# SLIDE-3D/SLIDE

Hardware: AMD Instinct MI355X
Metric: latent shapes/sec (pos+feat DDPM, 1000 steps, 16 pts) (higher is better)
Workload: dtype f16 (MFMA operands + activation storage; f32 accumulate, norm statistics, softmax); position DDPM: two-term f16 operand splits (fp32-grade); 1 GPU; BASELINE configs[1]+[2]: airplane position DDPM (16x3) + chair feature DDPM (16x51), batch 256 per GPU; 1 step = one reverse step of each; shape = 1000+1000 steps; batch_per_gpu=256, prec=fp16, pos_prec=split, replay=eager, pos_batch_multiple=2, pos_stream_cus=176, prime_steps=0, finite=True

## Files before the change

### slide_amd/csrc/ddpm_update.h

```cpp
#pragma once
#include "gemm_common.h"

namespace {

__device__ __forceinline__ void philox_round(uint32_t &c0, uint32_t &c1, uint32_t &c2, uint32_t &c3, uint32_t k0,
                                             uint32_t k1) {
  const uint64_t p0 = (uint64_t)0xD2511F53u * c0, p1 = (uint64_t)0xCD9E8D57u * c2;
  const uint32_t n0 = (uint32_t)(p1 >> 32) ^ c1 ^ k0, n1 = (uint32_t)p1, n2 = (uint32_t)(p0 >> 32) ^ c3 ^ k1,
                 n3 = (uint32_t)p0;
  c0 = n0; c1 = n1; c2 = n2; c3 = n3;
}
__device__ __forceinline__ float philox_normal(uint32_t seed_lo, uint32_t seed_hi, uint32_t step, uint32_t elem,
                                               uint32_t nonce) {
  uint32_t c0 = elem, c1 = step, c2 = 0x243F6A88u ^ nonce, c3 = 0x85A308D3u, k0 = seed_lo, k1 = seed_hi;
#pragma unroll
  for (int i = 0; i < 10; ++i) {
    philox_round(c0, c1, c2, c3, k0, k1);
    k0 += 0x9E3779B9u; k1 += 0xBB67AE85u;
  }
  const float u1 = ((float)(c0 >> 8) + 0.5f) * (1.0f / 16777216.0f);
  const float u2 = ((float)(c1 >> 8) + 0.5f) * (1.0f / 16777216.0f);
  return sqrtf(-2.0f * logf(u1)) * cosf(6.28318530717958647692f * u2);
}

__device__ __forceinline__ void advance_t_last_block(int *t_dev, int t, int step) {
  __syncthreads();
  if (threadIdx.x == 0) {
    __threadfence();
    if (atomicAdd(&t_dev[2], 1) == (int)gridDim.x - 1) {
      t_dev[2] = 0;
      t_dev[0] = t - 1;
      t_dev[1] = step + 1;
    }
  }
}

__device__ __forceinline__ void update_feat_element(int e, int npts, int C, int kdim, int eps_ld, float clamp,
                                                    uint32_t seed_lo, uint32_t seed_hi, float *__restrict__ x,
                                                    const float *__restrict__ eps, const float *__restrict__ noise, int t,
                                                    int step, uint32_t nonce, uint32_t eoff, const float *__restrict__ complete_x0,
                                                    const float *__restrict__ kmask, const float *__restrict__ keypoint,
                                                    const float *__restrict__ rc, const float *__restrict__ rm1,
                                                    const float *__restrict__ c1, const float *__restrict__ c2,
                                                    const float *__restrict__ stdv, void *__restrict__ feat0 = nullptr,
                                                    int ldf = 0, int half_out = 0,
                                                    const SlidePrepCopy *__restrict__ copies = nullptr, int n_copies = 0,
                                                    float eps_val = 0.f,
                                                    const float *z_pre = nullptr) {
#pragma clang fp contract(off)
  if (e >= npts * C) return;
  const int p = e / C, c = e - p * C;
  if (c < kdim) {
    x[e] = keypoint[(size_t)p * kdim + c];
    return;
  }
  const float xv = x[e];
  float x0 = rc[t] * xv - rm1[t] * (eps ? eps[eps_ld ? (size_t)p * eps_ld + c : (size_t)e] : eps_val);
  if (clamp > 0.f) x0 = fminf(fmaxf(x0, -clamp), clamp);
  if (complete_x0) {
    const float m = kmask[p];
    x0 = x0 * m + complete_x0[e] * (1.f - m);
  }
// ... 25 lines not shown
```

### slide_amd/csrc/engine.hip

```cpp
#include "gemm_common.h"
#include "gemm_small.h"
#include "ddpm_update.h"

#include <cstdlib>

int slide_launch_rows_op(const SlideOp &o, hipStream_t s);
#ifdef SLIDE_EXPERIMENTS
int slide_launch_gemm_xs(const GemmArgs &a, int npxl, int cbw, bool aff, bool gat, int want_occ, hipStream_t s);
#endif
int slide_launch_gemm_gx(const SlideOp &o, hipStream_t s);
int slide_launch_gemm_gxs(const SlideOp &o, hipStream_t s);
int slide_launch_attn_tail_split(const SlideOp &o, hipStream_t s);
int slide_launch_point_chain(const SlideOp &o, hipStream_t s);
int slide_launch_pp_stage(const SlideOp &o, hipStream_t s);
int slide_launch_pair_norm(const SlideOp &o, hipStream_t s);
int slide_launch_sa_chain(const SlideOp &o, hipStream_t s);
int slide_launch_block_body(const SlideOp &o, hipStream_t s);
#ifdef SLIDE_EXPERIMENTS
int slide_launch_gemm_chain(const SlideOp &o, hipStream_t s);
#endif
#define SLIDE_ST_EXPERIMENT (-20)
int slide_launch_gemm_gx_dual(const SlideOp &o, hipStream_t s);
int slide_launch_sa_chain_p(const SlideOp &o, hipStream_t s);

namespace {

template <int PREC, int NPXL, int CBW, bool PAIRRES = false>
__global__ __launch_bounds__(256, (PREC == SLIDE_PREC_SPLIT && NPXL == 4) ? 1 : 2) void gemm_kernel(GemmArgs a) {
  using T = typename TileT<PREC>::T;
  constexpr int LDK = TileT<PREC>::LDK;
  constexpr int EPL = TileT<PREC>::EPL;
  constexpr int TPR = BK / EPL;
  constexpr int RPP = 256 / TPR;
  constexpr int TN = 32 * CBW;
  constexpr int XP = TM / RPP, WP = TN / RPP;
  extern __shared__ __attribute__((aligned(16))) unsigned char smem_raw[];
  constexpr bool SPLIT = PREC == SLIDE_PREC_SPLIT;
// ... 1636 lines not shown
                  w3 = w[(size_t)(k + 3) * n_o + j], w4 = w[(size_t)(k + 4) * n_o + j], w5 = w[(size_t)(k + 5) * n_o + j],
                  w6 = w[(size_t)(k + 6) * n_o + j], w7 = w[(size_t)(k + 7) * n_o + j];
      a0 += in[k] * w0; a1 += in[k + 1] * w1_; a2 += in[k + 2] * w2_; a3 += in[k + 3] * w3;
      a0 += in[k + 4] * w4; a1 += in[k + 5] * w5; a2 += in[k + 6] * w6; a3 += in[k + 7] * w7;
    }
    return (a0 + a1) + (a2 + a3);
  };
  for (int j = tid; j < H; j += 256) h1[j] = swishf(b1[j] + gemv(emb, t_dim, w1, H, j));
  __syncthreads();
  for (int j = tid; j < H; j += 256) h2[j] = swishf(b2[j] + gemv(h1, H, w2, H, j));
  __syncthreads();
  for (int j = tid; j < n_out; j += 256) out[(size_t)b * n_out + j] = bfc[j] + gemv(h2, H, wfc, n_out, j);
}

__global__ __launch_bounds__(256) void cond_kernel(int dim, int n_out, const int64_t *__restrict__ label,
                                                   const float *__restrict__ class_emb, const float *__restrict__ wfc,
                                                   const float *__restrict__ bfc, float *__restrict__ out) {
  extern __shared__ float sm[];
  const int b = blockIdx.x, tid = threadIdx.x;
  const float *ce = class_emb + (size_t)label[b] * dim;
  for (int k = tid; k < dim; k += 256) sm[k] = ce[k];
  __syncthreads();
  for (int j = tid; j < n_out; j += 256) {
    float acc = bfc[j];
    for (int k = 0; k < dim; ++k) acc += sm[k] * wfc[(size_t)k * n_out + j];
    out[(size_t)b * n_out + j] = acc;
  }
}

__global__ __launch_bounds__(256) void update_pos_kernel(int n, int eps_ld, uint32_t seed_lo, uint32_t seed_hi, float *__restrict__ x,
                                                         const float *__restrict__ eps, const float *__restrict__ noise,
                                                         int *__restrict__ t_dev, const float *__restrict__ c_eps,
                                                         const float *__restrict__ sqrt_alpha,
                                                         const float *__restrict__ sigma) {
#pragma clang fp contract(off)
  const int e = blockIdx.x * 256 + threadIdx.x;
  const int t = t_dev[0], step = t_dev[1];
  if (e < n) {
    const int ep = eps_ld ? (e / 3) * eps_ld + e % 3 : e;
    float v = (x[e] - c_eps[t] * eps[ep]) / sqrt_alpha[t];
    if (t > 0) {
      const float z = noise ? noise[(size_t)step * n + e]
                            : philox_normal(seed_lo, seed_hi, (uint32_t)step, (uint32_t)e + (uint32_t)t_dev[4] * 48u, (uint32_t)t_dev[3]);
      v = v + sigma[t] * z;
    }
    x[e] = v;
  }
  advance_t_last_block(t_dev, t, step);
}

__global__ __launch_bounds__(256) void update_feat_kernel(int npts, int C, int kdim, int eps_ld, float clamp, uint32_t seed_lo,
                                                          uint32_t seed_hi, float *__restrict__ x,
                                                          const float *__restrict__ eps, const float *__restrict__ noise,
                                                          int *__restrict__ t_dev, const float *__restrict__ keypoint,
                                                          const float *__restrict__ rc, const float *__restrict__ rm1,
                                                          const float *__restrict__ c1, const float *__restrict__ c2,
                                                          const float *__restrict__ stdv,
                                                          const float *__restrict__ complete_x0,
                                                          const float *__restrict__ kmask, void *__restrict__ feat0, int ldf,
                                                          int half_out, const SlidePrepCopy *__restrict__ copies, int n_copies) {
#pragma clang fp contract(off)
  const int t = t_dev[0], step = t_dev[1];
  const uint32_t nonce = (uint32_t)t_dev[3];
  const uint32_t eoff = (uint32_t)t_dev[4] * (uint32_t)(16 * C);
#pragma unroll
  for (int j = 0; j < 4; ++j)
    update_feat_element(blockIdx.x * 1024 + j * 256 + threadIdx.x, npts, C, kdim, eps_ld, clamp, seed_lo, seed_hi, x, eps, noise,
                        t, step, nonce, eoff, complete_x0, kmask, keypoint, rc, rm1, c1, c2, stdv, feat0, ldf, half_out, copies,
                        n_copies);
  advance_t_last_block(t_dev, t, step);
}

typedef SlideHeadArgs HeadArgs;

template <int K0MAX>
__global__ __launch_bounds__(256, 2) void head_update_kernel(HeadArgs a) {
#pragma clang fp contract(off)
  using T = _Float16;
  constexpr int LDX = K0MAX + 8, LDH = 128 + 8;
  __shared__ __attribute__((aligned(16))) T xs[64 * LDX];
  __shared__ __attribute__((aligned(16))) T hs[64 * LDH];
  const int tid = threadIdx.x, lane = tid & 63, wave = tid >> 6, half = lane >> 5, col = lane & 31;
  const int row0 = blockIdx.x * 64;
  const int t = a.t_dev[0], step = a.t_dev[1];
  const uint32_t nonce = (uint32_t)a.t_dev[3];
  const uint32_t eoff = (uint32_t)a.t_dev[4] * (uint32_t)(16 * a.C);
  const int nk0 = a.k0 >> 4;
  f16x8 w0[K0MAX / 16];
  {
    const GLOBAL_AS T *wp = gptr<const T>((uint64_t)a.W0) + (size_t)(wave * 32 + col) * a.k0 + half * 8;
#pragma unroll
    for (int s2 = 0; s2 < K0MAX / 16; ++s2)
      if (s2 < nk0) w0[s2] = *(const GLOBAL_AS f16x8 *)(wp + s2 * 16);
  }
  const int cb2 = a.n1c == 2 ? (wave & 1) : 0, rb2 = a.n1c == 2 ? (wave >> 1) : wave;
  const bool l2 = rb2 < 2;
  f16x8 w1[8];
  if (l2) {
    const GLOBAL_AS T *wp = gptr<const T>((uint64_t)a.W1) + (size_t)(cb2 * 32 + col) * 128 + half * 8;
#pragma unroll
    for (int s2 = 0; s2 < 8; ++s2) w1[s2] = *(const GLOBAL_AS f16x8 *)(wp + s2 * 16);
  }
  {
// ... 302 lines not shown
    a.add_bs = (int)o.f[2];
    a.add_n = (int)o.f[3] >> 1;
    a.aff_relu = (int)o.f[3] & 1;
  }
  a.at_V = o.p[5]; a.at_out = o.p[6]; a.at_counts = (const int *)o.p[7]; a.at_vss = (const float *)o.p[8];
  a.rows = o.i[0]; a.x_ld = o.i[1]; a.k_pad = o.i[2]; a.n_cob = o.i[3]; a.in_bs = o.i[5];
  resolve_epi(a);
  const int K = o.i[4];
  a.at_ldv = o.i[6]; a.at_ldo = o.i[7]; a.at_pps = o.i[8] > 0 ? o.i[8] : 1; a.at_vrelu = o.i[9]; a.at_C = o.i[10];
  a.at_klog2 = K == 4 ? 2 : K == 8 ? 3 : K == 16 ? 4 : K == 32 ? 5 : -1;
  if (a.at_klog2 < 0 || a.rows <= 0 || a.rows % K || a.k_pad % BK || a.x_ld % 8 || a.n_cob <= 0 || !a.X || !a.W || !a.epi || !a.at_V ||
      !a.at_out || a.at_ldv % 4 || a.at_ldo % 4 || a.at_ldv < a.n_cob * 32 || a.at_ldo < a.n_cob * 32 || (a.in_scale && !a.in_shift))
    return -3;
  return a.in_scale ? launch_gemm_attend<true>(a, s) : launch_gemm_attend<false>(a, s);
}

int run_gemm(const SlideOp &o, hipStream_t s) {
  GemmArgs a;
  a.X = o.p[0]; a.W = o.p[1]; a.epi = (const SlideEpi *)o.p[2];
  a.in_scale = (const float *)o.p[3]; a.in_shift = (const float *)o.p[4];
  a.in_add = nullptr; a.aff_relu = 0; a.add_bs = 0; a.add_n = 0; a.aff_tps = 1;
  if (a.in_scale && !o.p[8]) {
    a.in_add = (const float *)o.p[11];
    a.aff_tps = (int)o.f[1] > 1 ? (int)o.f[1] : 1;
    a.add_bs = (int)o.f[2];
    a.add_n = (int)o.f[3] >> 1;
    a.aff_relu = (int)o.f[3] & 1;
  }
  a.dbg = (unsigned long long *)o.p[5];
  a.stagger = (int)(o.f[0] * 100.f);
  a.sched = (int *)o.p[7];
  a.gfeat = o.p[8]; a.gidx = (const int *)o.p[9];
  a.gn_fin = (const SlideGnFin *)o.p[6];
  a.gx_d2 = (const float *)o.p[12]; a.gx_w = (const float *)o.p[13];
  a.gx_ta = a.gx_tb = nullptr; a.gx_vv = nullptr; a.gx_add_idx = nullptr;
  a.g_nsplit = (int)o.f[1]; a.g_ldf = (int)o.f[2]; a.g_klog2 = (int)o.f[3];
  a.rows = o.i[0]; a.x_ld = o.i[1]; a.k_pad = o.i[2]; a.n_cob = o.i[3]; a.in_bs = o.i[5];
  a.ch_epi = nullptr; a.ch_n_cob = 0;
  resolve_epi(a);
  const int npxl = o.i[4], prec = o.i[6], cbw = o.i[7], glds = o.i[8] & 1;
  a.w_cm = (o.i[8] >> 1) & 1;
  if ((o.i[8] >> 2) & 1) {
    if (prec == SLIDE_PREC_SPLIT && !glds && !a.in_scale && !o.p[8] && !o.p[10] && cbw == 2) {
      if (a.k_pad % BK || a.x_ld % 4 || a.rows <= 0 || a.n_cob <= 0) return -3;
      if (npxl == 8) return launch_gemm<SLIDE_PREC_SPLIT, 8, 2, true>(a, s);
      if (npxl == 7) return launch_gemm<SLIDE_PREC_SPLIT, 7, 2, true>(a, s);
      return -12;
    }
    if (!glds || prec != SLIDE_PREC_F16 || a.in_scale || o.p[8] || o.p[10]) return -12;
    if (npxl == 8) return launch_gemm_glds<8, 2, 3, 32, false, false, true>(a, s);
    if (npxl == 7) return launch_gemm_glds<7, 2, 3, 32, false, false, true>(a, s);
    return -12;
  }
  if (a.w_cm && (!glds || (npxl != 7 && npxl != 8) || o.p[10] || o.i[9] == 1)) return -11;
  if (a.k_pad % BK || a.x_ld % 8 || a.rows <= 0 || a.n_cob <= 0) return -3;
  if (prec == SLIDE_PREC_F16 && npxl == 4 && o.i[9] != 3 &&
      (!a.gn_fin || ((a.rows + 63) / 64) * ((a.n_cob + 1) / 2) <= 1024))
    return launch_gemm_small(a, s);
  if (a.gn_fin) return -10;
#ifndef SLIDE_EXPERIMENTS
  if (o.p[10]) return SLIDE_ST_EXPERIMENT;
#else
  if (o.p[10] && glds && prec == SLIDE_PREC_F16 && o.i[9] != 5 && (npxl == 8 || npxl == 7) && !(a.gfeat && a.in_scale)) {
    int st = -8;
    const bool aff = a.in_scale != nullptr, gat = a.gfeat != nullptr;
    st = slide_launch_gemm_xs(a, npxl, cbw, aff, gat, o.i[9] >= 11 && o.i[9] <= 13 ? o.i[9] - 10 : 0, s);
// ... 234 lines not shown
                     (const TT *)o.p[0], (const TT *)o.p[1], (TT *)o.p[2])
      if (o.i[5] == 16 && o.i[6] == SLIDE_PREC_F16) ATTN(16, _Float16);
      else if (o.i[5] == 16) ATTN(16, float);
      else if (o.i[5] == 8 && o.i[6] == SLIDE_PREC_F16) ATTN(8, _Float16);
      else if (o.i[5] == 8) ATTN(8, float);
      else return -5;
#undef ATTN
      break;
    }
    case SLIDE_OP_COPY_COLS: {
      if (o.i[0] <= 0 || o.i[1] <= 0) break;
      const dim3 g((o.i[0] * o.i[1] + 255) / 256), blk(256);
#define CPY(TS, TD)                                                                                               \
  hipLaunchKernelGGL((copy_cols_kernel<TS, TD>), g, blk, 0, s, o.i[0], o.i[1], o.i[2], o.i[3], (const TS *)o.p[0], \
                     (TD *)o.p[1])
      if (o.i[4] && o.i[5]) CPY(_Float16, _Float16);
      else if (o.i[4]) CPY(_Float16, float);
      else if (o.i[5]) CPY(float, _Float16);
      else CPY(float, float);
#undef CPY
      break;
    }
    case SLIDE_OP_TEMB:
      hipLaunchKernelGGL(temb_kernel, dim3(o.i[0]), dim3(256), (size_t)o.i[1] * 9 * sizeof(float), s, o.i[1], o.i[2],
                         (const float *)o.p[0], (const int *)o.p[1], (const float *)o.p[9], (const float *)o.p[2],
                         (const float *)o.p[3], (const float *)o.p[4], (const float *)o.p[5], (const float *)o.p[6],
                         (const float *)o.p[7], (float *)o.p[8]);
      break;
    case SLIDE_OP_COND:
      hipLaunchKernelGGL(cond_kernel, dim3(o.i[0]), dim3(256), (size_t)o.i[1] * sizeof(float), s, o.i[1], o.i[2],
                         (const int64_t *)o.p[0], (const float *)o.p[1], (const float *)o.p[2], (const float *)o.p[3],
                         (float *)o.p[4]);
      break;
    case SLIDE_OP_UPDATE_POS:
      hipLaunchKernelGGL(update_pos_kernel, dim3((o.i[0] + 255) / 256), dim3(256), 0, s, o.i[0], o.i[1], (uint32_t)o.i[2],
                         (uint32_t)o.i[3], (float *)o.p[0], (const float *)o.p[1], (const float *)o.p[2],
                         (int *)o.p[3], (const float *)o.p[4], (const float *)o.p[5], (const float *)o.p[6]);
      break;
    case SLIDE_OP_UPDATE_FEAT:
      hipLaunchKernelGGL(update_feat_kernel, dim3((o.i[0] * o.i[1] + 1023) / 1024), dim3(256), 0, s, o.i[0], o.i[1],
                         o.i[2], o.i[5], o.f[0], (uint32_t)o.i[3], (uint32_t)o.i[4], (float *)o.p[0], (const float *)o.p[1],
                         (const float *)o.p[2], (int *)o.p[3], (const float *)o.p[4], (const float *)o.p[5],
                         (const float *)o.p[6], (const float *)o.p[7], (const float *)o.p[8], (const float *)o.p[9],
                         (const float *)o.p[10], (const float *)o.p[11], o.p[12], o.i[6], o.i[7],
                         (const SlidePrepCopy *)o.p[13], o.i[8]);
      break;
#ifndef SLIDE_EXPERIMENTS
    case SLIDE_OP_HEAD_UPDATE:
    case SLIDE_OP_GEMM_CHAIN:
      return SLIDE_ST_EXPERIMENT;
#else
    case SLIDE_OP_GEMM_CHAIN:
      return slide_launch_gemm_chain(o, s);
    case SLIDE_OP_HEAD_UPDATE: {
      const SlideHeadArgs *h = (const SlideHeadArgs *)o.p[0];
      if (!h || h->rows <= 0 || h->rows % 16 || h->k0 % 32 || h->k0 <= 0 || h->k0 > 160 || h->x_ld < h->k0 || h->x_ld % 8 ||
          (h->n1c != 1 && h->n1c != 2) || !h->X || !h->W0 || !h->W1 || !h->v0 || !h->b1 || !h->x || !h->t_dev ||
          (h->kind != 0 && h->kind != 1) || h->C > 32 * h->n1c)
        return -3;
      const int grid = (h->rows + 63) / 64;
      if (h->k0 <= 96) hipLaunchKernelGGL(head_update_kernel<96>, dim3(grid), dim3(256), 0, s, *h);
      else hipLaunchKernelGGL(head_update_kernel<160>, dim3(grid), dim3(256), 0, s, *h);
      break;
    }
#endif
    case SLIDE_OP_POINT_CHAIN:
      return slide_launch_point_chain(o, s);
    case SLIDE_OP_GEMM_ATTEND:
      return run_gemm_attend(o, s);
    case SLIDE_OP_ATTN_TAIL:
      return ((int)o.f[1] & 8) ? slide_launch_attn_tail_split(o, s) : run_attn_tail(o, s);
    case SLIDE_OP_GEMM_GX:
      return (int)o.f[0] == 3 ? slide_launch_gemm_gxs(o, s) : slide_launch_gemm_gx(o, s);
    case SLIDE_OP_GEMM_GX_DUAL:
      return slide_launch_gemm_gx_dual(o, s);
    case SLIDE_OP_PAIR_NORM:
      return slide_launch_pair_norm(o, s);
    case SLIDE_OP_PP_STAGE:
      return slide_launch_pp_stage(o, s);
// ... 163 lines not shown
```

### slide_amd/csrc/gemm_common.h

```cpp
#pragma once
#include <hip/hip_runtime.h>
#include <stdint.h>

#include <type_traits>

#include "../../include/slide_engine.h"

typedef float f32x16 __attribute__((ext_vector_type(16)));
typedef _Float16 f16x8 __attribute__((ext_vector_type(8)));
typedef _Float16 f16x4 __attribute__((ext_vector_type(4)));
typedef _Float16 f16x2 __attribute__((ext_vector_type(2)));
typedef uint32_t u32x4 __attribute__((ext_vector_type(4)));
typedef float f32x2 __attribute__((ext_vector_type(2)));

struct GemmArgs {
  const void *X;
  const void *W;
  const SlideEpi *epi;
  const float *in_scale, *in_shift;
  const float *in_add;
  int aff_relu, add_bs, add_n, aff_tps;
  int rows, x_ld, k_pad, n_cob, in_bs;
  int w_cm;
  int shm_bytes;
  const SlideGnFin *gn_fin;
  const void *gfeat;
  const int *gidx;
  int g_ldf, g_nsplit, g_klog2;
  int *sched;
  int stagger;
  unsigned long long *dbg;
  const void *gx_ta, *gx_tb;
  const float *gx_d2, *gx_w, *gx_vv;
  const int *gx_add_idx;
  int gx_ld, gx_mode, gx_add_idx_stride, gx_vbs;
  const void *ch_W;
  const SlideEpi *ch_epi;
  int ch_n_cob, ch_k_pad;
  const float *vecs, *ch_vecs;
  const void *at_V;
  void *at_out;
  const float *at_vss;
  const int *at_counts;
  int at_ldv, at_ldo, at_klog2, at_pps, at_vrelu, at_C;
};

static inline void resolve_epi(GemmArgs &a) {
  a.vecs = a.ch_vecs = nullptr;
  if ((uintptr_t)a.epi & SLIDE_EPI_PACKED_VECS) {
    a.epi = reinterpret_cast<const SlideEpi *>((uintptr_t)a.epi & ~SLIDE_EPI_PACKED_VECS);
    a.vecs = reinterpret_cast<const float *>(a.epi + a.n_cob);
  }
  if ((uintptr_t)a.ch_epi & SLIDE_EPI_PACKED_VECS) {
    a.ch_epi = reinterpret_cast<const SlideEpi *>((uintptr_t)a.ch_epi & ~SLIDE_EPI_PACKED_VECS);
    a.ch_vecs = reinterpret_cast<const float *>(a.ch_epi + a.ch_n_cob);
  }
}

// ... 789 lines not shown
```

### slide_amd/csrc/gemm_small.h

```cpp
#pragma once
#include "gemm_common.h"

namespace {

template <int NST, bool AFF, int PAIR>
__device__ __forceinline__ void small_body(const GemmArgs &a, const PairArgs &pa, const int bid) {
  using T = _Float16;
  constexpr int NPXL = 4;
  constexpr int STAGE_B = 96 * 64;
  constexpr int NJ = 6;
  extern __shared__ __attribute__((aligned(16))) unsigned char smem_raw[];
  SLIDE_STAMP(a, 0);
  const int ntc = (a.n_cob + 1) / 2;
  const int tc = bid % ntc, tr = bid / ntc;
  const int row0 = tr * 64, cob0 = tc * 2;
  const int tid = threadIdx.x, lane = tid & 63, wave = tid >> 6;
  const int half = lane >> 5, col = lane & 31;
  const int kh = wave >> 1, cbw = wave & 1;
  unsigned char *const ring = smem_raw + (size_t)wave * NST * STAGE_B;
  uint32_t *const epi_lds = reinterpret_cast<uint32_t *>(smem_raw + (size_t)4 * NST * STAGE_B);
  float *const vec_lds = reinterpret_cast<float *>(epi_lds + 2 * EPI_DW + (2 * EPI_DW) % 4);
  const T *gp[NJ];
#pragma unroll
  for (int j = 0; j < NJ; ++j) {
// ... 30 lines not shown
  }
  const int nk = a.k_pad / 32;
  const int mine = nk > kh ? (nk - kh + 1) / 2 : 0;
#pragma unroll
  for (int s0 = 0; s0 < NST - 1; ++s0)
    if (s0 < mine) issue(kh + 2 * s0, s0);
  stage_epilogue_tables<2>(a, cob0, tid, epi_lds, vec_lds);
  float *const pair_lds = vec_lds + 2 * 96;
  float *const pair_ext = reinterpret_cast<float *>(smem_raw + 20480);
  int ext_n[2] = {0, 0};
  float ext_d[2] = {0.f, 0.f}, ext_w[2] = {0.f, 0.f};
  if constexpr (PAIR != 0) {
    const int nb = a.rows >> NPXL, b0 = row0 >> NPXL;
    if (tid < 192) {
      const int bb = b0 + tid / 48 < nb ? b0 + tid / 48 : nb - 1;
      pair_lds[tid] = pa.xyz[(size_t)bb * 48 + tid % 48];
    }
    if (PAIR == 2) {
#pragma unroll
      for (int u = 0; u < 2; ++u) {
        const int i = tid + 256 * u;
        const int bb = b0 + (i >> 7) < nb ? b0 + (i >> 7) : nb - 1, t = i & 127;
        const int slot = (bb * 16 + (t >> 3)) * 16 + (t & 7);
        ext_n[u] = pa.nbr[slot]; ext_d[u] = pa.d2t[slot]; ext_w[u] = pa.wt[slot];
      }
    }
  }
  _Float16 *const aff_lds = reinterpret_cast<_Float16 *>(vec_lds + 2 * 96);
  if (AFF) {
    const int nb = a.rows >> NPXL;
    if (a.gn_fin) {
      const SlideGnFin f = *a.gn_fin;
      const int off = (int)(a.in_scale - f.scale);
      float *const grp = reinterpret_cast<float *>(aff_lds + (size_t)4 * 2 * a.k_pad);
      if (tid < 128) {
        const int sm = tid >> 5, g = tid & 31;
        int b = (row0 >> NPXL) + sm;
        b = b < nb ? b : nb - 1;
        float mean = 0.f, rstd = 0.f;
        if (g < f.G) {
#pragma clang fp contract(off)
          float S = 0.f, SS = 0.f;
          typedef float f4u __attribute__((ext_vector_type(4), aligned(4)));
          const int c_end = f.gend[g];
          const float *ps = f.sum + (size_t)b * f.bs, *pq = f.sq + (size_t)b * f.bs;
          for (int cc = f.gstart[g]; cc < c_end; cc += 16) {
            f4u s4[4], q4[4];
            int base[4];
#pragma unroll
            for (int u = 0; u < 4; ++u) {
              base[u] = cc + 4 * u + 4 <= f.bs ? cc + 4 * u : f.bs - 4;
              s4[u] = *reinterpret_cast<const f4u *>(ps + base[u]);
              q4[u] = *reinterpret_cast<const f4u *>(pq + base[u]);
            }
#pragma unroll
            for (int u = 0; u < 4; ++u)
#pragma unroll
              for (int e = 0; e < 4; ++e) {
                const int c = base[u] + e;
                if (c >= cc + 4 * u && c < c_end) { S += s4[u][e]; SS += q4[u][e]; }
              }
          }
          mean = S * f.inv_count;
          const float var = fmaxf(SS * f.inv_count - mean * mean, 0.f);
          rstd = 1.0f / sqrtf(var + GN_EPS);
        }
        grp[tid * 2] = mean;
        grp[tid * 2 + 1] = rstd;
      }
      __syncthreads();
      const int c_lo = tc == 0 ? 0 : off, c_n = tc == 0 ? f.C : (a.k_pad < f.C - off ? a.k_pad : f.C - off);
      for (int i0 = tid; i0 < 4 * c_n; i0 += 1024) {
        int gq[4];
        float gm[4], bt[4];
#pragma unroll
        for (int u = 0; u < 4; ++u) {
          const int i = i0 + 256 * u < 4 * c_n ? i0 + 256 * u : i0;
          const int c = c_lo + i % c_n;
          gq[u] = f.gid[c]; gm[u] = f.gamma[c]; bt[u] = f.beta[c];
        }
#pragma unroll
        for (int u = 0; u < 4; ++u) {
          const int i = i0 + 256 * u;
          if (i >= 4 * c_n) break;
          const int sm = i / c_n, c = c_lo + (i - sm * c_n);
          int b = (row0 >> NPXL) + sm;
          b = b < nb ? b : nb - 1;
          const int g = gq[u];
          float sc = 1.f, sh = 0.f;
          if (g >= 0) {
#pragma clang fp contract(off)
            sc = gm[u] * grp[(sm * 32 + g) * 2 + 1];
            sh = bt[u] - grp[(sm * 32 + g) * 2] * sc;
          }
          if (tc == 0) {
            f.scale[(size_t)b * f.bs + c] = sc;
            f.shift[(size_t)b * f.bs + c] = sh;
          }
          const int kk = c - off;
          if (kk >= 0 && kk < a.k_pad) {
            aff_lds[(sm * 2 + 0) * a.k_pad + kk] = (_Float16)sc;
            aff_lds[(sm * 2 + 1) * a.k_pad + kk] = (_Float16)sh;
          }
        }
      }
    } else {
      for (int i = tid; i < 4 * a.k_pad; i += 256) {
        const int sm = i / a.k_pad, k = i - sm * a.k_pad;
        int b = (row0 >> NPXL) + sm;
        b = b < nb ? b : nb - 1;
        aff_lds[(sm * 2 + 0) * a.k_pad + k] = (_Float16)a.in_scale[(size_t)b * a.in_bs + k];
        aff_lds[(sm * 2 + 1) * a.k_pad + k] = (_Float16)a.in_shift[(size_t)b * a.in_bs + k];
// ... 169 lines not shown
```

### slide_amd/diffusion.py

```python
import ctypes
import os
import weakref

import numpy as np
import torch

from ._lib import check, lib
from .abi import (OP_ADVANCE_T, OP_ATTN_TAIL, OP_GEMM, OP_HEAD_UPDATE, OP_POINT_CHAIN, OP_PREP_POINTS, OP_SYNC, OP_UPDATE_FEAT,
                  OP_UPDATE_POS, SlideHeadArgs, SlideOp, make_op)
from .engine import DenoiserEngine

F32 = np.float32


def calc_diffusion_hyperparams(T, beta_0, beta_T):
    start, end = F32(beta_0), F32(beta_T)
    step = F32((end - start) / F32(T - 1))
    i = np.arange(T)
    Beta = np.where(i < T // 2, float(start) + float(step) * i, float(end) - float(step) * (T - 1 - i)).astype(F32)
    Alpha = (F32(1) - Beta).astype(F32)
    Alpha_bar, Beta_tilde = Alpha.copy(), Beta.copy()
    for t in range(1, T):
        Alpha_bar[t] = F32(Alpha_bar[t] * Alpha_bar[t - 1])
        Beta_tilde[t] = F32(Beta_tilde[t] * F32(F32(1 - Alpha_bar[t - 1]) / F32(1 - Alpha_bar[t])))
# ... 68 lines not shown
        if os.environ.get("SLIDE_STREAM_PRIO"):
            pp = [int(v) for v in os.environ["SLIDE_STREAM_PRIO"].split(",")]
            prio = pp[0] if hp.get("in_fea_dim", 0) == 0 else pp[-1]
        if stream is not None:
            self.stream = stream
        else:
            self.stream = torch.cuda.Stream(device=device, priority=prio) if prio else torch.cuda.Stream(device=device)
        self._masked_stream, self.n_cus = None, 0
        if stream is not None:
            cu_share = 0.0
        env_cus = os.environ.get("SLIDE_POS_CUS" if hp.get("in_fea_dim", 0) == 0 else "SLIDE_FEAT_CUS")
        ncu = int(env_cus) if env_cus is not None else (
            int(torch.cuda.get_device_properties(device).multi_processor_count * cu_share) if (cu_share and device.type == "cuda") else 0)
        if ncu > 0 and device.type == "cuda":
            total = torch.cuda.get_device_properties(device).multi_processor_count
            first = int(os.environ.get("SLIDE_CU_MASK_FROM", "0"))
            words = [0] * ((total + 31) // 32)
            for cu in range(first, min(first + ncu, total)):
                words[cu // 32] |= 1 << (cu % 32)
            handle, key, st = _masked_stream_lease(device, tuple(words))
            if handle:
                self._masked_stream, self.n_cus = handle, min(first + ncu, total) - first
                self.stream = torch.cuda.ExternalStream(handle, device=device)
                weakref.finalize(self, _masked_stream_return, key, handle)
            else:
                import warnings
                warnings.warn("slide_stream_create_cu_mask failed (status %d): the chain runs on all compute units" % st)
        self.stream2 = torch.cuda.Stream(device=device) if self.engine.two_lanes else self.stream
        self.graph = None
        self.step_ops = None

    def _finish_plan(self, update_op, fixed_xyz=False):
        e = self.engine
        hoisted = set(e.xyz_copy_idx) if fixed_xyz else set()
        drop = hoisted | {e.eps_copy_idx}
        self.fuse_prep = False
        if (fixed_xyz and update_op.kind == OP_UPDATE_FEAT and os.environ.get("SLIDE_FUSE_PREP", "1") != "0"
                and e.ops[e._prep_idx].p[5] is None):
            prep = e.ops[e._prep_idx]
            assert prep.kind == OP_PREP_POINTS
            update_op.p[12] = e.feat0.data_ptr()
            update_op.i[6], update_op.i[7] = e.feat0.shape[1], int(e.feat0.dtype == torch.float16)
            update_op.p[13], update_op.i[8] = prep.p[6], prep.i[4]
            drop = drop | {e._prep_idx}
            self.fuse_prep = True
        head = getattr(e, "head", None)
        if (head is not None and os.environ.get("SLIDE_HEAD_UPDATE", "0") != "0" and update_op.kind in (OP_UPDATE_POS, OP_UPDATE_FEAT)
                and e.ops[head["idx"][0]].kind == OP_GEMM and e.ops[head["idx"][1]].kind == OP_GEMM and head["idx"][1] == e.eps_copy_idx - 1):
            h, u = SlideHeadArgs(), update_op
            h.X, h.W0, h.W1, h.v0, h.b1 = (head[k_].data_ptr() for k_ in ("X", "W0", "W1", "v0", "b1"))
            h.eps_out = None
            h.rows, h.x_ld, h.k0, h.n1c, h.eps_ld = self.B * 16, head["X"].shape[1], head["k0"], head["n1c"], e.eps_pad.shape[1]
            h.x, h.noise, h.t_dev = u.p[0], u.p[2], u.p[3]
            if u.kind == OP_UPDATE_POS:
                h.kind, h.C, h.kdim = 0, 3, 0
                h.seed_lo, h.seed_hi = u.i[2] & 0xFFFFFFFF, u.i[3] & 0xFFFFFFFF
                h.t0, h.t1, h.t2 = u.p[4], u.p[5], u.p[6]
            else:
                h.kind, h.C, h.kdim = 1, u.i[1], u.i[2]
                h.seed_lo, h.seed_hi = u.i[3] & 0xFFFFFFFF, u.i[4] & 0xFFFFFFFF
                h.clamp = u.f[0]
                h.keypoint, h.t0, h.t1, h.t2, h.t3, h.t4 = u.p[4], u.p[5], u.p[6], u.p[7], u.p[8], u.p[9]
                h.complete_x0, h.kmask = u.p[10], u.p[11]
                h.feat0, h.ldf, h.half_out, h.copies, h.n_copies = u.p[12], u.i[6], u.i[7], u.p[13], u.i[8]
            self._head_args = h
            update_op = make_op(OP_HEAD_UPDATE, p=(ctypes.addressof(h),))
# ... 369 lines not shown
```

### slide_amd/engine.py

```python
import ctypes
import os

import numpy as np
import torch

from ._lib import SlideHipError, check, lib
from .abi import *


def gn_layout(C):
    G = min(32, C)
    n_norm = C - C % G
    gs = n_norm // G
    gs_p = 1
    while gs_p < gs:
        gs_p *= 2
    assert gs_p <= 32, "GroupNorm group size > 32 not supported by the epilogue"
    idx = np.empty(C, np.int64)
    for c in range(C):
        idx[c] = (c // gs) * gs_p + c % gs if c < n_norm else G * gs_p + (c - n_norm)
    return idx, int(G * gs_p + (C - n_norm)), int(G * gs_p), int(gs_p), int(gs)


class _Arena:
# ... 291 lines not shown
        ntr = (rows + 255) // 256
        cbw = 4 if (self.prec == 1 and n_cob >= 4 and ntr * ((n_cob + 3) // 4) >= int(os.environ.get('SLIDE_CBW4_TILES', '1000'))) else 2
        if (self.prec == 1 and self.use_glds and sc is None and npx_log2 >= 7 and ntr * n_cob <= int(os.environ.get('SLIDE_CBW1_TILES', '0'))):
            cbw = 1
        self.gemm_flops[len(self.ops)] = 2 * rows * sum(int(s["w"].size) for s in segs)
        esz = X.element_size()
        rd = rows * ld * esz + W.size * esz + sum(rows * v[2] * esz for v in vec_list if v[1].get("residual") is not None)
        rd += sum((rows >> max(v[1]["pre_add"][1], 0) if v[1]["pre_add"][1] >= 0 else rows >> npx_log2 << 4) * v[2] * esz
                  for v in vec_list if v[1].get("pre_add") is not None)
        wr = sum(rows * v[2] * v[1]["out"].element_size() for v in vec_list)
        self.gemm_bytes[len(self.ops)] = (rd, wr)
        glds = int(self.use_glds and self.prec == 1 and (sc is None or npx_log2 >= 7))
        wfrag = None
        xs_mode = os.environ.get("SLIDE_XS", "")
        xs_levels = {7, 8} if xs_mode == "auto" else {int(v) for v in xs_mode.split(",") if v}
        xs_lds = ((ld - (gather[3] * 32 if gather is not None else 0)) // 32) * 16384
        if (glds and npx_log2 in xs_levels and gn_fin is None and not (gather is not None and sc is not None)
                and xs_lds + 20 * 1024 <= 160 * 1024):
            if xs_mode != "auto" or gather is not None or (npx_log2 == 8 and sc is None and n_cob >= 16 and xs_lds > 96 * 1024):
                wfrag = Wd
                cbw = 4 if n_cob >= 4 and os.environ.get("SLIDE_XS_CBW", "2") == "4" else 2
        gtab = None if gather is None else self._cm_copy.get(gather[0].data_ptr(), gather[0])
        assert wfrag is None or gtab is None or gtab is gather[0]
        gf = (0.0, 0.0, 0.0) if gather is None else (float(gather[3]), float(32 if gtab is not gather[0] else gather[0].shape[1]),
                                                     float({8: 3, 16: 4}[gather[2]]))
        knob = self.glds_nst
        assert wfrag is None or not (w_cm or self._is_cm(X))
        if wfrag is not None and os.environ.get("SLIDE_XS_OCC"):
            knob = 10 + int(os.environ["SLIDE_XS_OCC"])
        has_pair = any(v[1].get("res_pair") is not None for v in vec_list)
        if self.use_gxs and npx_log2 == 4 and gather is None and gn_fin is None and pre_gather is None and wfrag is None and \
                not any(v[1].get("pre_add") is not None for v in vec_list):
            self._w16_next = W
        self._emit(make_op(OP_GEMM, i=(rows, x_ld, ld, n_cob, npx_log2, in_bs, self.prec, cbw, glds | (2 if w_cm else 0) | (4 if has_pair else 0), knob),
                           f=(-1.0 if self.persistent == 2 else float(os.environ.get('SLIDE_STAGGER_US', '0')),) + gf,
                                p=(X.data_ptr(), Wd.data_ptr(), edp,
                                   None if sc is None else sc.data_ptr() + 4 * aff_off,
                                   None if sh is None else sh.data_ptr() + 4 * aff_off, None,
                                   None if gn_fin is None else gn_fin.data_ptr(),
                                   self._sched().data_ptr() if self.persistent else None,
                                   None if gather is None else gtab.data_ptr(),
                                   (None if pre_gather is None else pre_gather.data_ptr()) if gather is None
                                   else gather[1].data_ptr(),
                                   None if wfrag is None else wfrag.data_ptr(), None,
                                   None if pair_tabs is None else pair_tabs[1].data_ptr(),
                                   None if pair_tabs is None else pair_tabs[2].data_ptr())))
        if pair_tabs is not None:
            assert gather is None and pre_gather is None
            self.ops[-1].p[9] = pair_tabs[0].data_ptr()
        self.flops += 2 * rows * sum(int(s["w"].size) for s in segs)

    @staticmethod
    def _split1_ok(*ws):
        return all(float(np.abs(w).max()) < 31.0 for w in ws if w.size)

    def _emit_gx(self, gx, npx_log2, rows, ld, n_cob, Wd, edp, segs, W, vec_list, in_affine, pair_tabs, chain=None, keep=None):
        ta, tb, coff = gx["ta"], gx["tb"], gx["coff"]
        tes = ta.element_size()
        assert ta.dtype == (torch.float16 if self.prec == 1 else torch.float32) and ta.shape == tb.shape and coff % 8 == 0
        assert ta.shape[1] >= coff + ld
        fl = 2 * rows * sum(int(s_["w"].size) for s_ in segs)
        self.gemm_flops[len(self.ops)] = fl
        rd = 2 * (rows >> npx_log2) * 16 * ld * tes + W.size * tes
        wr = sum(rows * v[2] * v[1]["out"].element_size() for v in vec_list if v[1]["out"] is not None)
        if chain is not None:
            fl += chain["flops"]; rd += chain["wbytes"]; wr += chain["wr"]
            self.gemm_flops[len(self.ops)] = fl
# ... 1165 lines not shown
```

Measured before the change: 424.0 shapes/s.

## Add early-signal DDPM update kernels and packed GroupNorm-finish stat staging

Adds update_pos/feat 'early' kernels. They load all operands and compute the new values first, then bump the step counter with an acq_rel atomic and no threadfence before issuing the stores. This shortens the serialized tail of each reverse step. Separately, the GEMM GroupNorm-finish prologue now stages per-batch sum and sum-of-squares into LDS via global_load_lds and prefetches gamma, beta and gid into registers, in place of strided global reads. Both are on by default through environment flags. Timeline stamp instrumentation is added but compiled out.

```diff
diff --git a/slide_amd/csrc/ddpm_update.h b/slide_amd/csrc/ddpm_update.h
--- a/slide_amd/csrc/ddpm_update.h
+++ b/slide_amd/csrc/ddpm_update.h
@@ -2,6 +2,21 @@
 #include "gemm_common.h"
 
 namespace {
+
+#ifdef SLIDE_TIMELINE
+#define UPD_STAMP(k, dep)                                                                    \
+  do {                                                                                       \
+    asm volatile("" ::"v"(dep));                                                             \
+    if (dbg && threadIdx.x == 0) dbg[(size_t)blockIdx.x * 16 + (k)] = wall_clock64();       \
+  } while (0)
+#define UPD_STAMP_RETIRED(k)                                                                 \
+  do {                                                                                       \
+    if (dbg) { asm volatile("s_waitcnt vmcnt(0)" ::: "memory"); UPD_STAMP(k, 0); }           \
+  } while (0)
+#else
+#define UPD_STAMP(k, dep) do { } while (0)
+#define UPD_STAMP_RETIRED(k) do { } while (0)
+#endif
 
 __device__ __forceinline__ void philox_round(uint32_t &c0, uint32_t &c1, uint32_t &c2, uint32_t &c3, uint32_t k0,
                                              uint32_t k1) {
@@ -23,11 +38,14 @@
   return sqrtf(-2.0f * logf(u1)) * cosf(6.28318530717958647692f * u2);
 }
 
-__device__ __forceinline__ void advance_t_last_block(int *t_dev, int t, int step) {
+__device__ __forceinline__ void advance_t_last_block(int *t_dev, int t, int step, unsigned long long *dbg = nullptr) {
   __syncthreads();
+  UPD_STAMP(5, 0);
   if (threadIdx.x == 0) {
     __threadfence();
-    if (atomicAdd(&t_dev[2], 1) == (int)gridDim.x - 1) {
+    const int done = atomicAdd(&t_dev[2], 1);
+    UPD_STAMP(6, done);
+    if (done == (int)gridDim.x - 1) {
       t_dev[2] = 0;
       t_dev[0] = t - 1;
       t_dev[1] = step + 1;
diff --git a/slide_amd/csrc/engine.hip b/slide_amd/csrc/engine.hip
--- a/slide_amd/csrc/engine.hip
+++ b/slide_amd/csrc/engine.hip
@@ -3,6 +3,7 @@
 #include "ddpm_update.h"
 
 #include <cstdlib>
+#include <cstring>
 
 int slide_launch_rows_op(const SlideOp &o, hipStream_t s);
 #ifdef SLIDE_EXPERIMENTS
@@ -1705,10 +1706,12 @@
                                                          const float *__restrict__ eps, const float *__restrict__ noise,
                                                          int *__restrict__ t_dev, const float *__restrict__ c_eps,
                                                          const float *__restrict__ sqrt_alpha,
-                                                         const float *__restrict__ sigma) {
+                                                         const float *__restrict__ sigma, unsigned long long *dbg) {
 #pragma clang fp contract(off)
+  UPD_STAMP(0, 0);
   const int e = blockIdx.x * 256 + threadIdx.x;
   const int t = t_dev[0], step = t_dev[1];
+  UPD_STAMP(1, t + step);
   if (e < n) {
     const int ep = eps_ld ? (e / 3) * eps_ld + e % 3 : e;
     float v = (x[e] - c_eps[t] * eps[ep]) / sqrt_alpha[t];
@@ -1719,7 +1722,9 @@
     }
     x[e] = v;
   }
-  advance_t_last_block(t_dev, t, step);
+  UPD_STAMP(7, 0);
+  UPD_STAMP_RETIRED(8);
+  advance_t_last_block(t_dev, t, step, dbg);
 }
 
 __global__ __launch_bounds__(256) void update_feat_kernel(int npts, int C, int kdim, int eps_ld, float clamp, uint32_t seed_lo,
@@ -1731,9 +1736,12 @@
                                                           const float *__restrict__ stdv,
                                                           const float *__restrict__ complete_x0,
                                                           const float *__restrict__ kmask, void *__restrict__ feat0, int ldf,
-                                                          int half_out, const SlidePrepCopy *__restrict__ copies, int n_copies) {
+                                                          int half_out, const SlidePrepCopy *__restrict__ copies, int n_copies,
+                                                          unsigned long long *dbg) {
 #pragma clang fp contract(off)
+  UPD_STAMP(0, 0);
   const int t = t_dev[0], step = t_dev[1];
+  UPD_STAMP(1, t + step);
   const uint32_t nonce = (uint32_t)t_dev[3];
   const uint32_t eoff = (uint32_t)t_dev[4] * (uint32_t)(16 * C);
 #pragma unroll
@@ -1741,7 +1749,157 @@
     update_feat_element(blockIdx.x * 1024 + j * 256 + threadIdx.x, npts, C, kdim, eps_ld, clamp, seed_lo, seed_hi, x, eps, noise,
                         t, step, nonce, eoff, complete_x0, kmask, keypoint, rc, rm1, c1, c2, stdv, feat0, ldf, half_out, copies,
                         n_copies);
-  advance_t_last_block(t_dev, t, step);
+  UPD_STAMP(7, 0);
+  UPD_STAMP_RETIRED(8);
+  advance_t_last_block(t_dev, t, step, dbg);
+}
+
+__device__ __forceinline__ void advance_t_counted(int *t_dev, int t, int step, unsigned long long *dbg) {
+  if (threadIdx.x == 0) {
+    const int done = __hip_atomic_fetch_add(&t_dev[2], 1, __ATOMIC_ACQ_REL, __HIP_MEMORY_SCOPE_AGENT);
+    UPD_STAMP(6, done);
+    if (done == (int)gridDim.x - 1) {
+      t_dev[2] = 0;
+      t_dev[0] = t - 1;
+      t_dev[1] = step + 1;
+    }
+  }
+}
+
+__global__ __launch_bounds__(256) void update_pos_early_kernel(int n, int eps_ld, uint32_t seed_lo, uint32_t seed_hi,
+                                                               float *__restrict__ x, const float *__restrict__ eps,
+                                                               const float *__restrict__ noise, int *__restrict__ t_dev,
+                                                               const float *__restrict__ c_eps, const float *__restrict__ sqrt_alpha,
+                                                               const float *__restrict__ sigma, unsigned long long *dbg) {
+#pragma clang fp contract(off)
+  UPD_STAMP(0, 0);
+  const int e = blockIdx.x * 256 + threadIdx.x;
+  const bool live = e < n;
+  const int t = t_dev[0], step = t_dev[1];
+  const uint32_t nonce = (uint32_t)t_dev[3], eoff = (uint32_t)t_dev[4] * 48u;
+  float xv = 0.f, ev = 0.f;
+  if (live) {
+    const int ep = eps_ld ? (e / 3) * eps_ld + e % 3 : e;
+    xv = x[e];
+    ev = eps[ep];
+  }
+  UPD_STAMP(1, t + step);
+  const float k_eps = c_eps[t], k_sa = sqrt_alpha[t], k_sg = sigma[t];
+  float z = 0.f;
+  if (live && t > 0)
+    z = noise ? noise[(size_t)step * n + e] : philox_normal(seed_lo, seed_hi, (uint32_t)step, (uint32_t)e + eoff, nonce);
+  UPD_STAMP(2, k_eps + k_sa + k_sg);
+  float v = (xv - k_eps * ev) / k_sa;
+  UPD_STAMP(3, v);
+  if (t > 0) v = v + k_sg * z;
+  UPD_STAMP(4, v);
+  __syncthreads();
+  UPD_STAMP(5, 0);
+  advance_t_counted(t_dev, t, step, dbg);
+  if (live) x[e] = v;
+  UPD_STAMP(7, 0);
+  UPD_STAMP_RETIRED(8);
+}
+
+constexpr int UPD_MAX_COPIES = 8;
+
+__global__ __launch_bounds__(256) void update_feat_early_kernel(int npts, int C, int kdim, int eps_ld, float clamp, uint32_t seed_lo,
+                                                                uint32_t seed_hi, float *__restrict__ x,
+                                                                const float *__restrict__ eps, const float *__restrict__ noise,
+                                                                int *__restrict__ t_dev, const float *__restrict__ keypoint,
+                                                                const float *__restrict__ rc, const float *__restrict__ rm1,
+                                                                const float *__restrict__ c1, const float *__restrict__ c2,
+                                                                const float *__restrict__ stdv,
+                                                                const float *__restrict__ complete_x0,
+                                                                const float *__restrict__ kmask, void *__restrict__ feat0, int ldf,
+                                                                int half_out, const SlidePrepCopy *__restrict__ copies, int n_copies,
+                                                                unsigned long long *dbg) {
+#pragma clang fp contract(off)
+  UPD_STAMP(0, 0);
+  const int t = t_dev[0], step = t_dev[1];
+  const uint32_t nonce = (uint32_t)t_dev[3];
+  const uint32_t eoff = (uint32_t)t_dev[4] * (uint32_t)(16 * C);
+  void *cp_dst[UPD_MAX_COPIES];
+  int cp_ld[UPD_MAX_COPIES], cp_n[UPD_MAX_COPIES];
+#pragma unroll
+  for (int q = 0; q < UPD_MAX_COPIES; ++q) {
+    cp_dst[q] = nullptr; cp_ld[q] = 0; cp_n[q] = 0;
+    if (feat0 && q < n_copies) {
+      const SlidePrepCopy d = copies[q];
+      cp_dst[q] = d.dst; cp_ld[q] = d.ld; cp_n[q] = d.kind == 0 ? d.n : 0;
+    }
+  }
+  const int n = npts * C;
+  int pp[4], cc[4];
+  bool live[4], key[4];
+  float xv[4], ev[4], cx[4], mk[4];
+#pragma unroll
+  for (int j = 0; j < 4; ++j) {
+    const int e = blockIdx.x * 1024 + j * 256 + threadIdx.x;
+    live[j] = e < n;
+    pp[j] = e / C; cc[j] = e - pp[j] * C;
+    key[j] = cc[j] < kdim;
+    xv[j] = ev[j] = cx[j] = 0.f; mk[j] = 1.f;
+    if (live[j]) {
+      if (key[j]) {
+        xv[j] = keypoint[(size_t)pp[j] * kdim + cc[j]];
+      } else {
+        xv[j] = x[e];
+        if (eps) ev[j] = eps[eps_ld ? (size_t)pp[j] * eps_ld + cc[j] : (size_t)e];
+        if (complete_x0) { cx[j] = complete_x0[e]; mk[j] = kmask[pp[j]]; }
+      }
+    }
+  }
+  UPD_STAMP(1, t + step);
+  const float k_rc = rc[t], k_rm1 = rm1[t], k_c1 = c1[t], k_c2 = c2[t], k_std = stdv[t];
+  float z[4];
+#pragma unroll
+  for (int j = 0; j < 4; ++j) {
+    z[j] = 0.f;
+    if (t > 0 && live[j] && !key[j]) {
+      const int e = blockIdx.x * 1024 + j * 256 + threadIdx.x;
+      z[j] = noise ? noise[(size_t)step * npts * C + e] : philox_normal(seed_lo, seed_hi, (uint32_t)step, (uint32_t)e + eoff, nonce);
+    }
+  }
+  UPD_STAMP(2, k_rc + k_rm1 + k_c1 + k_c2 + k_std);
+  float v[4];
+#pragma unroll
+  for (int j = 0; j < 4; ++j) {
+    float x0 = k_rc * xv[j] - k_rm1 * ev[j];
+    if (clamp > 0.f) x0 = fminf(fmaxf(x0, -clamp), clamp);
+    if (complete_x0) x0 = x0 * mk[j] + cx[j] * (1.f - mk[j]);
+    v[j] = k_c1 * x0 + k_c2 * xv[j];
+  }
+  UPD_STAMP(3, v[0] + v[1] + v[2] + v[3]);
+#pragma unroll
+  for (int j = 0; j < 4; ++j) {
+    if (t > 0) v[j] = v[j] + k_std * z[j];
+    if (key[j]) v[j] = xv[j];
+  }
+  UPD_STAMP(4, v[0] + v[1] + v[2] + v[3]);
+  __syncthreads();
+  UPD_STAMP(5, 0);
+  advance_t_counted(t_dev, t, step, dbg);
+#pragma unroll
+  for (int j = 0; j < 4; ++j) {
+    if (!live[j]) continue;
+    const int e = blockIdx.x * 1024 + j * 256 + threadIdx.x;
+    x[e] = v[j];
+    if (feat0 && !key[j]) {
+      const int cf = cc[j] - kdim;
+      const size_t p = (size_t)pp[j];
+      if (half_out) reinterpret_cast<_Float16 *>(feat0)[p * ldf + cf] = (_Float16)v[j];
+      else reinterpret_cast<float *>(feat0)[p * ldf + cf] = v[j];
+#pragma unroll
+      for (int q = 0; q < UPD_MAX_COPIES; ++q)
+        if (cf < cp_n[q]) {
+          if (half_out) reinterpret_cast<_Float16 *>(cp_dst[q])[p * cp_ld[q] + cf] = (_Float16)v[j];
+          else reinterpret_cast<float *>(cp_dst[q])[p * cp_ld[q] + cf] = v[j];
+        }
+    }
+  }
+  UPD_STAMP(7, 0);
+  UPD_STAMP_RETIRED(8);
 }
 
 typedef SlideHeadArgs HeadArgs;
@@ -2110,6 +2268,7 @@
   a.sched = (int *)o.p[7];
   a.gfeat = o.p[8]; a.gidx = (const int *)o.p[9];
   a.gn_fin = (const SlideGnFin *)o.p[6];
+  a.fin_packed = (o.i[8] >> 3) & 1;
   a.gx_d2 = (const float *)o.p[12]; a.gx_w = (const float *)o.p[13];
   a.gx_ta = a.gx_tb = nullptr; a.gx_vv = nullptr; a.gx_add_idx = nullptr;
   a.g_nsplit = (int)o.f[1]; a.g_ldf = (int)o.f[2]; a.g_klog2 = (int)o.f[3];
@@ -2410,19 +2569,31 @@
                          (const int64_t *)o.p[0], (const float *)o.p[1], (const float *)o.p[2], (const float *)o.p[3],
                          (float *)o.p[4]);
       break;
-    case SLIDE_OP_UPDATE_POS:
-      hipLaunchKernelGGL(update_pos_kernel, dim3((o.i[0] + 255) / 256), dim3(256), 0, s, o.i[0], o.i[1], (uint32_t)o.i[2],
+    case SLIDE_OP_UPDATE_POS: {
+      unsigned long long *dbg = nullptr;
+#ifdef SLIDE_TIMELINE
+      dbg = (unsigned long long *)o.p[7];
+#endif
+      auto *kern = (o.i[4] & 1) ? update_pos_early_kernel : update_pos_kernel;
+      hipLaunchKernelGGL(kern, dim3((o.i[0] + 255) / 256), dim3(256), 0, s, o.i[0], o.i[1], (uint32_t)o.i[2],
                          (uint32_t)o.i[3], (float *)o.p[0], (const float *)o.p[1], (const float *)o.p[2],
-                         (int *)o.p[3], (const float *)o.p[4], (const float *)o.p[5], (const float *)o.p[6]);
+                         (int *)o.p[3], (const float *)o.p[4], (const float *)o.p[5], (const float *)o.p[6], dbg);
       break;
-    case SLIDE_OP_UPDATE_FEAT:
-      hipLaunchKernelGGL(update_feat_kernel, dim3((o.i[0] * o.i[1] + 1023) / 1024), dim3(256), 0, s, o.i[0], o.i[1],
+    }
+    case SLIDE_OP_UPDATE_FEAT: {
+      unsigned long long *dbg = nullptr;
+#ifdef SLIDE_TIMELINE
+      memcpy(&dbg, &o.f[2], sizeof(dbg));
+#endif
+      auto *kern = ((o.i[9] & 1) && o.i[8] <= UPD_MAX_COPIES) ? update_feat_early_kernel : update_feat_kernel;
+      hipLaunchKernelGGL(kern, dim3((o.i[0] * o.i[1] + 1023) / 1024), dim3(256), 0, s, o.i[0], o.i[1],
                          o.i[2], o.i[5], o.f[0], (uint32_t)o.i[3], (uint32_t)o.i[4], (float *)o.p[0], (const float *)o.p[1],
                          (const float *)o.p[2], (int *)o.p[3], (const float *)o.p[4], (const float *)o.p[5],
                          (const float *)o.p[6], (const float *)o.p[7], (const float *)o.p[8], (const float *)o.p[9],
                          (const float *)o.p[10], (const float *)o.p[11], o.p[12], o.i[6], o.i[7],
-                         (const SlidePrepCopy *)o.p[13], o.i[8]);
+                         (const SlidePrepCopy *)o.p[13], o.i[8], dbg);
       break;
+    }
 #ifndef SLIDE_EXPERIMENTS
     case SLIDE_OP_HEAD_UPDATE:
     case SLIDE_OP_GEMM_CHAIN:
diff --git a/slide_amd/csrc/gemm_common.h b/slide_amd/csrc/gemm_common.h
--- a/slide_amd/csrc/gemm_common.h
+++ b/slide_amd/csrc/gemm_common.h
@@ -24,6 +24,7 @@
   int w_cm;
   int shm_bytes;
   const SlideGnFin *gn_fin;
+  int fin_packed;
   const void *gfeat;
   const int *gidx;
   int g_ldf, g_nsplit, g_klog2;
diff --git a/slide_amd/csrc/gemm_small.h b/slide_amd/csrc/gemm_small.h
--- a/slide_amd/csrc/gemm_small.h
+++ b/slide_amd/csrc/gemm_small.h
@@ -86,7 +86,41 @@
     if (a.gn_fin) {
       const SlideGnFin f = *a.gn_fin;
       const int off = (int)(a.in_scale - f.scale);
+#ifdef SLIDE_TIMELINE
+      asm volatile("" ::"s"(f.bs));
+      SLIDE_STAMP(a, 12);
+#endif
       float *const grp = reinterpret_cast<float *>(aff_lds + (size_t)4 * 2 * a.k_pad);
+      const int c_lo = tc == 0 ? 0 : off, c_n = tc == 0 ? f.C : (a.k_pad < f.C - off ? a.k_pad : f.C - off);
+      const bool packed = a.fin_packed && f.bs * 8 <= STAGE_B;
+      int pk_gs = 0, pk_ge = 0, pk_gq[4] = {-1, -1, -1, -1};
+      float pk_gm[4] = {0.f, 0.f, 0.f, 0.f}, pk_bt[4] = {0.f, 0.f, 0.f, 0.f};
+      if (packed) {
+        const int w = __builtin_amdgcn_readfirstlane(wave);
+        int b = (row0 >> NPXL) + w;
+        b = b < nb ? b : nb - 1;
+        float *const dst = reinterpret_cast<float *>(smem_raw + ((size_t)w * NST + (NST - 1)) * STAGE_B);
+        const float *ps = f.sum + (size_t)b * f.bs, *pq = f.sq + (size_t)b * f.bs;
+        for (int i0 = 0; i0 < f.bs; i0 += 64)
+          if (i0 + lane < f.bs) {
+            __builtin_amdgcn_global_load_lds((const GLOBAL_AS void *)(ps + i0 + lane),
+                                             (__attribute__((address_space(3))) void *)(dst + i0), 4, 0, 0);
+            __builtin_amdgcn_global_load_lds((const GLOBAL_AS void *)(pq + i0 + lane),
+                                             (__attribute__((address_space(3))) void *)(dst + f.bs + i0), 4, 0, 0);
+          }
+        if (tid < 128 && (tid & 31) < f.G) { pk_gs = f.gstart[tid & 31]; pk_ge = f.gend[tid & 31]; }
+        if (tid < 4 * c_n) {
+#pragma unroll
+          for (int u = 0; u < 4; ++u) {
+            const int i = tid + 256 * u < 4 * c_n ? tid + 256 * u : tid;
+            const int c = c_lo + i % c_n;
+            pk_gq[u] = f.gid[c]; pk_gm[u] = f.gamma[c]; pk_bt[u] = f.beta[c];
+          }
+        }
+        asm volatile("s_waitcnt vmcnt(0)" ::: "memory");
+        __syncthreads();
+        SLIDE_STAMP(a, 13);
+      }
       if (tid < 128) {
         const int sm = tid >> 5, g = tid & 31;
         int b = (row0 >> NPXL) + sm;
@@ -95,6 +129,10 @@
         if (g < f.G) {
 #pragma clang fp contract(off)
           float S = 0.f, SS = 0.f;
+          if (packed) {
+            const float *rs = reinterpret_cast<const float *>(smem_raw + ((size_t)sm * NST + (NST - 1)) * STAGE_B);
+            for (int c = pk_gs; c < pk_ge; ++c) { S += rs[c]; SS += rs[f.bs + c]; }
+          } else {
           typedef float f4u __attribute__((ext_vector_type(4), aligned(4)));
           const int c_end = f.gend[g];
           const float *ps = f.sum + (size_t)b * f.bs, *pq = f.sq + (size_t)b * f.bs;
@@ -115,6 +153,7 @@
                 if (c >= cc + 4 * u && c < c_end) { S += s4[u][e]; SS += q4[u][e]; }
               }
           }
+          }
           mean = S * f.inv_count;
           const float var = fmaxf(SS * f.inv_count - mean * mean, 0.f);
           rstd = 1.0f / sqrtf(var + GN_EPS);
@@ -123,7 +162,7 @@
         grp[tid * 2 + 1] = rstd;
       }
       __syncthreads();
-      const int c_lo = tc == 0 ? 0 : off, c_n = tc == 0 ? f.C : (a.k_pad < f.C - off ? a.k_pad : f.C - off);
+      SLIDE_STAMP(a, 14);
       for (int i0 = tid; i0 < 4 * c_n; i0 += 1024) {
         int gq[4];
         float gm[4], bt[4];
@@ -131,7 +170,8 @@
         for (int u = 0; u < 4; ++u) {
           const int i = i0 + 256 * u < 4 * c_n ? i0 + 256 * u : i0;
           const int c = c_lo + i % c_n;
-          gq[u] = f.gid[c]; gm[u] = f.gamma[c]; bt[u] = f.beta[c];
+          if (packed && i0 == tid) { gq[u] = pk_gq[u]; gm[u] = pk_gm[u]; bt[u] = pk_bt[u]; }
+          else { gq[u] = f.gid[c]; gm[u] = f.gamma[c]; bt[u] = f.beta[c]; }
         }
 #pragma unroll
         for (int u = 0; u < 4; ++u) {
diff --git a/slide_amd/diffusion.py b/slide_amd/diffusion.py
--- a/slide_amd/diffusion.py
+++ b/slide_amd/diffusion.py
@@ -124,6 +124,8 @@
 
     def _finish_plan(self, update_op, fixed_xyz=False):
         e = self.engine
+        if os.environ.get("SLIDE_UPDATE_EARLY", "1") != "0":
+            update_op.i[9 if update_op.kind == OP_UPDATE_FEAT else 4] |= 1
         hoisted = set(e.xyz_copy_idx) if fixed_xyz else set()
         drop = hoisted | {e.eps_copy_idx}
         self.fuse_prep = False
diff --git a/slide_amd/engine.py b/slide_amd/engine.py
--- a/slide_amd/engine.py
+++ b/slide_amd/engine.py
@@ -347,7 +347,8 @@
         if self.use_gxs and npx_log2 == 4 and gather is None and gn_fin is None and pre_gather is None and wfrag is None and \
                 not any(v[1].get("pre_add") is not None for v in vec_list):
             self._w16_next = W
-        self._emit(make_op(OP_GEMM, i=(rows, x_ld, ld, n_cob, npx_log2, in_bs, self.prec, cbw, glds | (2 if w_cm else 0) | (4 if has_pair else 0), knob),
+        fin_packed = 8 if (gn_fin is not None and os.environ.get("SLIDE_FIN_PACKED", "1") != "0") else 0
+        self._emit(make_op(OP_GEMM, i=(rows, x_ld, ld, n_cob, npx_log2, in_bs, self.prec, cbw, glds | (2 if w_cm else 0) | (4 if has_pair else 0) | fin_packed, knob),
                            f=(-1.0 if self.persistent == 2 else float(os.environ.get('SLIDE_STAGGER_US', '0')),) + gf,
                                 p=(X.data_ptr(), Wd.data_ptr(), edp,
                                    None if sc is None else sc.data_ptr() + 4 * aff_off,
```

New measurement: 423.6 shapes/s (median of 2 runs). About the same (-0.1%).
